# 2gunsu/monocon-pytorch

Hardware: AMD Instinct MI355X
Metric: images/sec (384x1280) fwd+bwd (higher is better)
Workload: dtype f32 (f16x2); 1 GPU; train step B=32/GPU 3x384x1280 (configs[2] shape, fp32 values, mode f16x2); global_batch=32, parallelism=dp1, precision_mode=f16x2

## Files before the change

### monocon-pytorch_amd/csrc/conv_mfma.h

```cpp
#pragma once
#include <hip/hip_runtime.h>
#include <stdint.h>
#include <atomic>
#include <type_traits>
#include <utility>

namespace mc {

typedef float f32x16 __attribute__((ext_vector_type(16)));
typedef float f32x4 __attribute__((ext_vector_type(4)));

struct DynLdsOnce {
    std::atomic<unsigned long long> done{0};
    hipError_t ensure(const void *fn, int bytes) {
        int dev = 0;
        if (hipGetDevice(&dev) != hipSuccess || dev < 0 || dev >= 64) return hipFuncSetAttribute(fn, hipFuncAttributeMaxDynamicSharedMemorySize, bytes);
        if ((done.load(std::memory_order_acquire) >> dev) & 1ull) return hipSuccess;
        const hipError_t e = hipFuncSetAttribute(fn, hipFuncAttributeMaxDynamicSharedMemorySize, bytes);
        if (e == hipSuccess) done.fetch_or(1ull << dev, std::memory_order_release);
        return e;
    }
};

struct ConvSrc {
// ... 324 lines not shown
        if (s.id == (cfg & CFG_SHAPE_BITS)) return s;
    return {0, 0, 0, 0, 0};
}
template <int I>
struct ConvShapeC {
    static constexpr int WM = CONV_SHAPES[I].WM, WN = CONV_SHAPES[I].WN, WTM = CONV_SHAPES[I].WTM, WTN = CONV_SHAPES[I].WTN;
    static constexpr int PB = CONV_SHAPES[I].PB(), BNT = CONV_SHAPES[I].BNT();
};
template <typename F, int... I>
inline hipError_t with_conv_shape_seq(int id, F &f, std::integer_sequence<int, I...>) {
    hipError_t e = hipErrorInvalidValue;
    (void)((CONV_SHAPES[I].id == id && ((e = f(ConvShapeC<I>{})), true)) || ...);
    return e;
}
template <typename F>
inline hipError_t with_conv_shape(int cfg, F &&f) {
    return with_conv_shape_seq(cfg & CFG_SHAPE_BITS, f, std::make_integer_sequence<int, CONV_NSHAPES>{});
}
template <int KS_, int S_>
struct ConvWin { static constexpr int KS = KS_, S = S_; };
template <typename F>
inline hipError_t with_conv_window(int ks, int stride, F &&f) {
    if (ks == 3 && stride == 1) return f(ConvWin<3, 1>{});
    if (ks == 3 && stride == 2) return f(ConvWin<3, 2>{});
    if (stride != 1) return hipErrorInvalidValue;
    if (ks == 1) return f(ConvWin<1, 1>{});
    if (ks == 12) return f(ConvWin<12, 1>{});
    if (ks == 21) return f(ConvWin<21, 1>{});
    if (ks == 22) return f(ConvWin<22, 1>{});
    return hipErrorInvalidValue;
}

template <auto Kern, typename... Args>
inline hipError_t launch_dyn_lds(size_t lds_bytes, dim3 grid, dim3 block, hipStream_t st, const Args &...args) {
    if (lds_bytes > 160 * 1024) return hipErrorInvalidValue;
    static DynLdsOnce attr_set;
    const hipError_t e = attr_set.ensure(reinterpret_cast<const void *>(Kern), (int)lds_bytes);
    if (e != hipSuccess) return e;
    hipLaunchKernelGGL(Kern, grid, block, lds_bytes, st, args...);
    return hipGetLastError();
}

inline int conv_ntile(int Cout) { return Cout >= 128 ? 128 : (Cout > 32 ? 64 : 32); }
inline int conv_coutp(int Cout) {
    const int t = conv_ntile(Cout);
    return (Cout + t - 1) / t * t;
}
inline int conv_out_dim(int in, int ks, int stride) { return (in + 2 * (ks / 2) - ks) / stride + 1; }
inline int split_pieces(int prec) { return prec == 2 ? 3 : (prec == 3 ? 2 : 1); }
inline int conv_ck(int ks, int stride, const int *src_c, int nsrc) {
    bool all32 = true;
    for (int i = 0; i < nsrc; ++i) all32 = all32 && (src_c[i] % 32 == 0);
    if (ks == 3 && stride == 2) return 16;
    return all32 ? 32 : 16;
}
int conv_pick_cfg(int Cout, int CoutP, int ks, int stride, int B, int Hout, int Wout);
inline int conv_chunks_per_image(int cfg, int Hout, int Wout) {
    if (cfg == CFG_SMALL) return Hout;
    return ((Wout + 7) / 8) * ((Hout + 3) / 4);
}
inline void conv_set_patches(ConvArgs &a, int PB) {
    a.ppr = (a.Wout + 7) / 8;
    a.ppi = a.ppr * ((a.Hout + 3) / 4);
    a.chunks = (a.ppi + PB - 1) / PB;
}
inline bool any_lazy_src(const ConvSrc *src, int nsrc) {
    for (int i = 0; i < nsrc; ++i)
        if (src[i].la) return true;
    return false;
}
inline bool conv_any_lazy(const ConvArgs &a) { return any_lazy_src(a.src, a.nsrc); }
bool conv_small_ok(const ConvArgs &a, int ks, int stride);
bool conv_small_lazy_ok(const ConvArgs &a, int ks, int stride);
bool conv_bf16_ok(const ConvArgs &a, int ks, int stride);
hipError_t launch_conv_bf16(const ConvArgs &a, int ks, int stride, hipStream_t st, ConvArgs *resolved);
hipError_t launch_absmax(const float *x, size_t n, unsigned *slot, hipStream_t st, bool single_word = false);
bool conv_wres_ok(const ConvArgs &a, int ks, int stride);
hipError_t launch_conv_wres(const ConvArgs &a, int ks, int stride, hipStream_t st, ConvArgs *resolved);
hipError_t launch_conv_small(const ConvArgs &a, int stride, hipStream_t st);
bool conv_thin_ok(const ConvArgs &a, int ks, int stride);
hipError_t launch_conv_thin(const ConvArgs &a, hipStream_t st);
bool dgrad_s2_thin_ok(int prec, int ks, int stride, int dyC, int srcC, int CinTotal, int c_off, const unsigned *amax_dy,
                      const unsigned *amax_w, int H, int W);
hipError_t launch_dgrad_s2_thin(const float *dy, int B, int H, int W, int dyC, const float *w_master, int CinTotal, int c_off, float *out,
                                int accumulate, const unsigned *amax_dy, const unsigned *amax_w, hipStream_t st);

hipError_t launch_conv(const ConvArgs &a, int ks, int stride, hipStream_t st, ConvArgs *resolved = nullptr);
bool conv_lazy_capable(const ConvArgs &a, int ks, int stride);

struct ProfLast { int kind; double flops, bytes; };
extern thread_local ProfLast prof_last;

}
```

### monocon-pytorch_amd/csrc/conv_thin.hip

```cpp
#include "conv_mfma.h"
#include "train.h"

#ifndef THIN_OCC
#define THIN_OCC 2
#endif
#ifndef THIN_MT_UNROLL
#define THIN_MT_UNROLL 1
#endif
namespace mc {

typedef _Float16 f16x8 __attribute__((ext_vector_type(8)));
typedef _Float16 f16x4 __attribute__((ext_vector_type(4)));
typedef float f32x4v __attribute__((ext_vector_type(4)));

namespace {
constexpr int TR = 8, TW = 64;
constexpr int IR = TR + 2, IP = TW + 2;
constexpr int PLANE = IR * IP * 16;
constexpr int ITEMS = IR * IP * 4;
constexpr int NI = (ITEMS + 255) / 256;
}

template <int NTN>
__global__ __launch_bounds__(256, THIN_OCC) void conv_thin16_kernel(const ConvArgs a) {
// ... 175 lines not shown
                            const unsigned char *p = lds + half * PLANE + ((trow + r) * IP + mt * 16 + li + c) * 16;
                            ah = *reinterpret_cast<const f16x8 *>(p);
                            al = *reinterpret_cast<const f16x8 *>(p + 2 * PLANE);
                        }
#pragma unroll
                        for (int nt = 0; nt < NTN; ++nt) {
                            accm[nt] = __builtin_amdgcn_mfma_f32_16x16x32_f16(al, bw[s][0][nt], accm[nt], 0, 0, 0);
                            accm[nt] = __builtin_amdgcn_mfma_f32_16x16x32_f16(ah, bw[s][1][nt], accm[nt], 0, 0, 0);
                            acc[nt] = __builtin_amdgcn_mfma_f32_16x16x32_f16(ah, bw[s][0][nt], acc[nt], 0, 0, 0);
                        }
                    }
#pragma unroll
                    for (int nt = 0; nt < NTN; ++nt) {
                        const int n = nt * 16 + li;
                        const int v_out = nok[nt] ? ((4 * kq) * a.out_ld + a.out_coff + n) * 4 : BUF_OOB;
                        const int v_res = nok[nt] ? ((4 * kq) * a.res_ld + n) * 4 : BUF_OOB;
                        float rv[4];
                        if (has_res) {
#pragma unroll
                            for (int e = 0; e < 4; ++e) rv[e] = buf_load1(r_res[q], v_res, (x0 + e) * a.res_ld * 4);
                        }
#pragma unroll
                        for (int e = 0; e < 4; ++e) {
                            float v = ((accm[nt][e] + acc[nt][e]) * omul) * sc[nt] + bi[nt];
                            if (has_res) v += rv[e];
                            if (bm) {
                                if (rok && nok[nt]) {
                                    const float yv = ybm[nt][e];
                                    const bool on = bm_relu == 0 || (bm_relu == 1 ? zbm[nt][e] > 0.f : fmaf(yv, ma[nt], mb[nt]) > 0.f);
                                    v = on ? v : 0.f;
                                    ssum[q][nt] += v;
                                    ssq[q][nt] = fmaf(v, yv, ssq[q][nt]);
                                }
                            } else if (do_stats) {
                                const float d = v - sh[nt];
                                ssum[q][nt] += d;
                                ssq[q][nt] += d * d;
                            }
                            v = fmaxf(v, floor_v);
                            vmax = fmaxf(vmax, (nok[nt] && oy0 + trow < a.Hout) ? fabsf(v) : 0.f);
                            buf_store1(v, r_out[q], v_out, (x0 + e) * a.out_ld * 4);
                        }
                    }
                }
            }
        }
        if (do_stats) {
#pragma unroll
            for (int q = 0; q < 2; ++q) {
                const int oy = oy0 + 2 * wave + q;
                if (oy >= a.Hout) continue;
#pragma unroll
                for (int nt = 0; nt < NTN; ++nt) {
                    float s1 = ssum[q][nt], s2 = ssq[q][nt];
                    s1 += __shfl_xor(s1, 16); s2 += __shfl_xor(s2, 16);
                    s1 += __shfl_xor(s1, 32); s2 += __shfl_xor(s2, 32);
                    if (kq == 0 && nok[nt]) {
                        float *dst = a.stats + (((size_t)img * a.Hout + oy) * a.CoutP + nt * 16 + li) * 2;
                        dst[0] = s1;
                        dst[1] = s2;
                    }
                }
            }
        }
    }
    if (a.amax_out) amax_update_wave(a.amax_out, vmax);
}

bool conv_thin_ok(const ConvArgs &a, int ks, int stride) {
#ifdef MC_NO_CONV_THIN
    return false;
#endif
    return a.prec == 3 && ks == 3 && stride == 1 && a.nsrc == 1 && a.Cin == 16 && a.Cout == 16 && a.amax_in[0] && a.amax_w &&
           a.Wout % 16 == 0 && a.Hout == a.Hin && a.Wout == a.Win && a.CoutP >= 16;
}

hipError_t launch_conv_thin(const ConvArgs &a, hipStream_t st) {
    const int tiles = a.B * ((a.Hout + TR - 1) / TR);
    hipLaunchKernelGGL((conv_thin16_kernel<1>), dim3(tiles < 4096 ? tiles : 4096), dim3(256), 0, st, a);
    return hipGetLastError();
}


struct DgradS2Args {
    const float *dy;
    const float *w;
    float *out;
    int B, H, W, CinTotal, c_off, accumulate;
    const unsigned *amax_dy, *amax_w;
};
namespace {
constexpr int DR = 4, DW = 32;
constexpr int DIR_ = DR + 1, DIP = DW + 1;
constexpr int DPLANE = DIR_ * DIP * 16;
}
template <int KS, int NT>
__global__ __launch_bounds__(256, KS == 1 ? 2 : 1) void dgrad_s2_thin_kernel(const DgradS2Args a) {
    constexpr int CY = 32 * KS, CX = 16 * NT, NOCT = 4 * KS;
    constexpr int DITEMS = DIR_ * DIP * (CY / 4), DNI = (DITEMS + 255) / 256;
    __shared__ __attribute__((aligned(16))) unsigned char lds[2 * NOCT * DPLANE];
    const int tid = threadIdx.x, lane = tid & 63;
    const int wave = __builtin_amdgcn_readfirstlane(tid >> 6);
    const int li = lane & 15, kq = lane >> 4;
    const int nt = wave % NT, row0 = (wave / NT) * NT;
    const int ex = f16_scale_exp(amax_read(a.amax_dy)), ew = f16_scale_exp(*a.amax_w);
    const float x_scale = exp2i(ex), w_scale = exp2i(ew), omul = exp2i(-ex) * exp2i(-ew);
    f16x8 bw[9][KS][2];
#pragma unroll
    for (int tap = 0; tap < 9; ++tap)
#pragma unroll
        for (int ks = 0; ks < KS; ++ks) {
            f16x8 h8, l8;
#pragma unroll
            for (int q = 0; q < 8; ++q) {
                const float ws = a.w[((size_t)(32 * ks + 8 * kq + q) * a.CinTotal + a.c_off + 16 * nt + li) * 9 + tap] * w_scale;
                const _Float16 hh = (_Float16)ws;
                h8[q] = hh;
                l8[q] = (_Float16)(ws - (float)hh);
            }
            bw[tap][ks][0] = h8; bw[tap][ks][1] = l8;
        }
    int s_off[DNI], s_dst[DNI];
#pragma unroll
    for (int i = 0; i < DNI; ++i) {
        const int e = tid + 256 * i;
        const int c4 = e % (CY / 4), px = (e / (CY / 4)) % DIP, row = (e / (CY / 4)) / DIP;
        s_off[i] = ((row * a.W + px) * CY + c4 * 4) * 4;
        s_dst[i] = e < DITEMS ? (c4 >> 1) * DPLANE + (row * DIP + px) * 16 + (c4 & 1) * 8 : -1;
    }
    const int tiles_per_img = (a.H + DR - 1) / DR, nstrips = (a.W + DW - 1) / DW;
    const int Ho = 2 * a.H, Wo = 2 * a.W;
    for (int tile = xcd_order(blockIdx.x, gridDim.x); tile < a.B * tiles_per_img; tile += gridDim.x) {
        const int img = tile / tiles_per_img, i0 = (tile - img * tiles_per_img) * DR;
        const __amdgpu_buffer_rsrc_t r_x = make_rsrc(a.dy + (size_t)img * a.H * a.W * CY, (unsigned)(a.H * a.W * CY) * 4u);
        __amdgpu_buffer_rsrc_t r_out[NT][2];
#pragma unroll
        for (int rr = 0; rr < NT; ++rr)
#pragma unroll
            for (int py = 0; py < 2; ++py) {
                const int i = i0 + row0 + rr;
                const bool ok = i < a.H;
                r_out[rr][py] = make_rsrc(a.out + ((size_t)img * Ho + (ok ? 2 * i + py : 0)) * Wo * CX, ok ? (unsigned)(Wo * CX) * 4u : 0u);
            }
        f32x4 pre[DNI];
        auto fetch = [&](int strip) {
            const int j0 = strip * DW, so = (i0 * a.W + j0) * CY * 4;
#pragma unroll
            for (int k = 0; k < DNI; ++k) {
                const int px = ((s_dst[k] % DPLANE) >> 4) % DIP;
                const bool ok = s_dst[k] >= 0 && j0 + px < a.W;
                pre[k] = buf_load4(r_x, ok ? s_off[k] + so : BUF_OOB, 0);
            }
        };
        fetch(0);
        for (int strip = 0; strip < nstrips; ++strip) {
            __syncthreads();
#pragma unroll
            for (int k = 0; k < DNI; ++k) {
                if (256 * (k + 1) > DITEMS && s_dst[k] < 0) continue;
                f16x4 h4, l4;
#pragma unroll
                for (int q = 0; q < 4; ++q) {
                    const float xs = pre[k][q] * x_scale;
                    const _Float16 hh = (_Float16)xs;
                    h4[q] = hh;
                    l4[q] = (_Float16)(xs - (float)hh);
                }
                *reinterpret_cast<f16x4 *>(lds + s_dst[k]) = h4;
                *reinterpret_cast<f16x4 *>(lds + NOCT * DPLANE + s_dst[k]) = l4;
            }
            __syncthreads();
            if (strip + 1 < nstrips) fetch(strip + 1);
            const int j0 = strip * DW;
#pragma unroll
            for (int rr = 0; rr < NT; ++rr) {
#pragma unroll
                for (int mt = 0; mt < DW / 16; ++mt) {
                    if (j0 + mt * 16 >= a.W) break;
#pragma unroll
                    for (int py = 0; py < 2; ++py) {
#pragma unroll
                        for (int px = 0; px < 2; ++px) {
                            f32x4v acc = {0.f, 0.f, 0.f, 0.f}, accm = {0.f, 0.f, 0.f, 0.f};
#pragma unroll
                            for (int dr = 0; dr <= py; ++dr) {
#pragma unroll
                                for (int ds = 0; ds <= px; ++ds) {
                                    const int r = py ? 2 - 2 * dr : 1, sx = px ? 2 - 2 * ds : 1, tap = r * 3 + sx;
#pragma unroll
                                    for (int ks = 0; ks < KS; ++ks) {
                                        const unsigned char *p = lds + (ks * 4 + kq) * DPLANE + ((row0 + rr + dr) * DIP + mt * 16 + li + ds) * 16;
                                        const f16x8 ah = *reinterpret_cast<const f16x8 *>(p), al = *reinterpret_cast<const f16x8 *>(p + NOCT * DPLANE);
                                        accm = __builtin_amdgcn_mfma_f32_16x16x32_f16(al, bw[tap][ks][0], accm, 0, 0, 0);
                                        accm = __builtin_amdgcn_mfma_f32_16x16x32_f16(ah, bw[tap][ks][1], accm, 0, 0, 0);
                                        acc = __builtin_amdgcn_mfma_f32_16x16x32_f16(ah, bw[tap][ks][0], acc, 0, 0, 0);
                                    }
                                }
                            }
#pragma unroll
                            for (int e = 0; e < 4; ++e) {
                                const int j = j0 + mt * 16 + 4 * kq + e;
                                const int voff = j < a.W ? ((2 * j + px) * CX + 16 * nt + li) * 4 : BUF_OOB;
                                float v = (accm[e] + acc[e]) * omul;
                                if (a.accumulate) v += buf_load1(r_out[rr][py], voff, 0);
                                buf_store1(v, r_out[rr][py], voff, 0);
                            }
                        }
                    }
                }
            }
        }
    }
}
bool dgrad_s2_thin_ok(int prec, int ks, int stride, int dyC, int srcC, int CinTotal, int c_off, const unsigned *amax_dy,
                      const unsigned *amax_w, int H, int W) {
    const bool shape = dyC == 32 && srcC == 16;
    return prec == 3 && ks == 3 && stride == 2 && shape && c_off >= 0 && c_off + srcC <= CinTotal && amax_dy && amax_w &&
           (size_t)H * W * dyC * 4 < (1ull << 31) && (size_t)4 * W * srcC * 4 < (1ull << 31);
}
hipError_t launch_dgrad_s2_thin(const float *dy, int B, int H, int W, int dyC, const float *w_master, int CinTotal, int c_off, float *out,
                                int accumulate, const unsigned *amax_dy, const unsigned *amax_w, hipStream_t st) {
    DgradS2Args a;
    a.dy = dy; a.w = w_master; a.out = out; a.B = B; a.H = H; a.W = W; a.CinTotal = CinTotal; a.c_off = c_off;
    a.accumulate = accumulate; a.amax_dy = amax_dy; a.amax_w = amax_w;
    const int tiles = B * ((H + DR - 1) / DR);
    const int srcC = dyC / 2;
    prof_last = {1, 2.0 * B * H * W * (double)dyC * srcC * 9.0, 4.0 * ((double)B * H * W * dyC + (double)B * 4 * H * W * srcC * (accumulate ? 2 : 1))};
    if (dyC != 32) return hipErrorInvalidValue;
    hipLaunchKernelGGL((dgrad_s2_thin_kernel<1, 1>), dim3(tiles < 4096 ? tiles : 4096), dim3(256), 0, st, a);
    return hipGetLastError();
}

namespace {
constexpr int WT_XT = 128, WT_P = 152, WT_ROWS = 6;
constexpr int WT_PLANE = 16 * WT_ROWS * WT_P * 2;
typedef unsigned u32x4 __attribute__((ext_vector_type(4)));
typedef _Float16 f16x2 __attribute__((ext_vector_type(2)));
}

__global__ __launch_bounds__(256) void wgrad_thin16_kernel(const WgradArgs a) {
    extern __shared__ __attribute__((aligned(16))) unsigned char wsm[];
    unsigned char *win = wsm;
    float (*red)[64] = reinterpret_cast<float (*)[64]>(wsm + 2 * WT_PLANE);
    const int tid = threadIdx.x, lane = tid & 63;
    const int wave = __builtin_amdgcn_readfirstlane(tid >> 6);
    const int g = lane >> 4, j = lane & 15;
    const int ex = f16_scale_exp(amax_read(a.amax_x[0])), ed = f16_scale_exp(amax_read(a.amax_dy));
    const float x_scale = exp2i(ex), d_scale = exp2i(ed), omul = exp2i(-ex) * exp2i(-ed);
    const int H = a.Hout, W = a.Wout;
    const bool lazy = a.src[0].la != nullptr;
    f32x4 lzA = {0.f, 0.f, 0.f, 0.f}, lzB = lzA;
    if (lazy) {
        lzA = reinterpret_cast<const f32x4 *>(a.src[0].la)[tid & 3];
        lzB = reinterpret_cast<const f32x4 *>(a.src[0].lb)[tid & 3];
#pragma unroll
        for (int q = 0; q < 4; ++q) { lzA[q] *= x_scale; lzB[q] *= x_scale; }
    }
    const unsigned x_bytes = (unsigned)(a.Hin * a.Win * 16) * 4u;
    unsigned okm = 0u;

    f32x4v acc[9], accm[9];
#pragma unroll
    for (int t = 0; t < 9; ++t) { acc[t] = f32x4v{0.f, 0.f, 0.f, 0.f}; accm[t] = f32x4v{0.f, 0.f, 0.f, 0.f}; }
    const int va = (8 * g * 16 + j) * 4;
    const int boff = ((j * WT_ROWS + wave) * WT_P + 8 * g) * 2;

    constexpr int NITEM = WT_ROWS * (WT_P / 2) * 4, NIW = (NITEM + 255) / 256;
    int w_off[NIW], w_dst[NIW];
#pragma unroll
    for (int i = 0; i < NIW; ++i) {
        const int e = tid + 256 * i, c4 = e & 3, pr = (e >> 2) % (WT_P / 2), row = (e >> 2) / (WT_P / 2);
        w_off[i] = ((row * a.Win + 2 * pr) * 16 + c4 * 4) * 4;
        w_dst[i] = e < NITEM ? ((c4 * 4 * WT_ROWS + row) * WT_P + 2 * pr) * 2 : -1;
    }
    const int tiles_x = (W + WT_XT - 1) / WT_XT, tiles_y = (H + 3) / 4;
    const int ntiles = a.B * tiles_y * tiles_x;
    f32x4 pv[NIW][2];
    auto fetch = [&](int tl) {
        const int b = tl / (tiles_y * tiles_x), rem = tl - b * tiles_y * tiles_x;
        const int y0 = (rem / tiles_x) * 4, x0 = (rem % tiles_x) * WT_XT;
        const __amdgpu_buffer_rsrc_t r_x = make_rsrc(a.src[0].p + (size_t)b * a.Hin * a.Win * 16, (unsigned)(a.Hin * a.Win * 16) * 4u);
        const int so = ((y0 - 1) * a.Win + x0 - 1) * 64;
        okm = 0u;
#pragma unroll
        for (int i = 0; i < NIW; ++i) {
            const int col = x0 - 1 + ((w_dst[i] >> 1) % WT_P);
            const bool live = w_dst[i] >= 0;
            const int vo0 = (live && col >= 0 && col < a.Win) ? w_off[i] + so : BUF_OOB;
            const int vo1 = (live && col + 1 >= 0 && col + 1 < a.Win) ? w_off[i] + so + 64 : BUF_OOB;
            pv[i][0] = buf_load4(r_x, vo0, 0);
            pv[i][1] = buf_load4(r_x, vo1, 0);
            if (lazy) okm |= (((unsigned)vo0 < x_bytes ? 1u : 0u) | ((unsigned)vo1 < x_bytes ? 2u : 0u)) << (2 * i);
        }
    };
    float araw[WT_XT / 32][8];
    auto fetch_dy = [&](int tl, float (&dst)[WT_XT / 32][8]) {
        const int b = tl / (tiles_y * tiles_x), rem = tl - b * tiles_y * tiles_x;
        const int y = (rem / tiles_x) * 4 + wave, x0 = (rem % tiles_x) * WT_XT;
        const __amdgpu_buffer_rsrc_t r_dy =
            make_rsrc(a.dy + ((size_t)b * H + (y < H ? y : 0)) * W * a.dy_ld, y < H ? (unsigned)(W * a.dy_ld) * 4u : 0u);
#pragma unroll
        for (int G = 0; G < WT_XT / 32; ++G)
#pragma unroll
            for (int t = 0; t < 8; ++t) dst[G][t] = buf_load1(r_dy, va + t * 64, (x0 + G * 32) * 64);
    };
    if ((int)blockIdx.x < ntiles) { fetch(blockIdx.x); fetch_dy(blockIdx.x, araw); }
    for (int tl = blockIdx.x; tl < ntiles; tl += gridDim.x) {
        __syncthreads();
#pragma unroll
        for (int i = 0; i < NIW; ++i) {
            if (w_dst[i] < 0) continue;
            const float cap0 = ((okm >> (2 * i)) & 1u) ? __builtin_inff() : 0.f, cap1 = ((okm >> (2 * i + 1)) & 1u) ? __builtin_inff() : 0.f;
// ... 94 lines not shown
```

### monocon-pytorch_amd/csrc/mc_train_plan.hip

```cpp
#include <atomic>
#include <deque>
#include <functional>

#include "mc_internal.h"

using namespace mc;

namespace {

using Fn = std::function<int(mc_handle *, hipStream_t)>;

struct PlanSwitches {
    long long lazy_z;
    long long lazy_min;
    long long lazy_feat;
    long long zbits;
    long long grad_pool;
    long long grad_pool_cool;
    long long head_dx_fuse;
    long long head_zskip;
    long long dgrad_s2_thin;
    long long stem_fuse;
    long long bm_epilogue;
    long long wres_bwd;
    long long dual_stream;
    int side_sync_lo = 0, side_sync_hi = 0;
    bool plan_debug = false;
};
const struct { const char *name; long long PlanSwitches::*field; long long def; } SWITCH_TABLE[] = {
    {"MONOCON_HIP_LAZY_Z", &PlanSwitches::lazy_z, 3},
    {"MONOCON_HIP_LAZY_MIN", &PlanSwitches::lazy_min, 900000},
    {"MONOCON_HIP_LAZY_FEAT", &PlanSwitches::lazy_feat, 0},
    {"MONOCON_HIP_ZBITS", &PlanSwitches::zbits, 1},
    {"MONOCON_HIP_GRAD_POOL", &PlanSwitches::grad_pool, 1},
    {"MONOCON_HIP_GRAD_POOL_COOL", &PlanSwitches::grad_pool_cool, 2},
    {"MONOCON_HIP_HEAD_DX_FUSE", &PlanSwitches::head_dx_fuse, 1},
    {"MONOCON_HIP_HEAD_ZSKIP", &PlanSwitches::head_zskip, 1},
    {"MONOCON_HIP_DGRAD_S2_THIN", &PlanSwitches::dgrad_s2_thin, 1},
    {"MONOCON_HIP_STEM_FUSE", &PlanSwitches::stem_fuse, 1},
    {"MONOCON_HIP_BM_EPILOGUE", &PlanSwitches::bm_epilogue, 1},
    {"MONOCON_HIP_WRES_BWD", &PlanSwitches::wres_bwd, 0},
    {"MONOCON_HIP_DUAL_STREAM", &PlanSwitches::dual_stream, 1},
};
PlanSwitches read_switches() {
    PlanSwitches sw{};
    std::string changed;
    for (const auto &d : SWITCH_TABLE) {
        const char *e = std::getenv(d.name);
        sw.*d.field = e ? std::atoll(e) : d.def;
        if (sw.*d.field != d.def) changed += std::string(" ") + d.name + "=" + std::to_string(sw.*d.field);
    }
    if (const char *e = std::getenv("MONOCON_HIP_SIDE_SYNC")) {
        if (std::sscanf(e, "%d:%d", &sw.side_sync_lo, &sw.side_sync_hi) != 2) sw.side_sync_lo = sw.side_sync_hi = 0;
        if (sw.side_sync_lo < sw.side_sync_hi) changed += std::string(" MONOCON_HIP_SIDE_SYNC=") + e;
    }
    sw.plan_debug = std::getenv("MONOCON_HIP_PLAN_DEBUG") != nullptr;
    if (sw.plan_debug && !changed.empty()) fprintf(stderr, "[plan] switches off their defaults:%s\n", changed.c_str());
    return sw;
}

struct PoolBwdArgs {
    const float *x, *dout, *la, *lb;
    float *dx, *stats;
    int B, H, W, C, acc;
};

struct LastWriter {
    enum Kind { NONE, DGRAD_CONV, POOL_BWD, DECONV_BWD } kind = NONE;
    union {
        ConvArgs *conv;
        PoolBwdArgs *pool;
        float **deconv_stats;
    };
    LastWriter() : conv(nullptr) {}
    LastWriter(ConvArgs *c) : kind(c ? DGRAD_CONV : NONE), conv(c) {}
    LastWriter(PoolBwdArgs *p) : kind(p ? POOL_BWD : NONE), pool(p) {}
    LastWriter(float **s) : kind(s ? DECONV_BWD : NONE), deconv_stats(s) {}
};

struct TNode {
    Tensor t;
    float *g = nullptr;
    bool ginit = false, needs_grad = true;
    LastWriter last;
};

enum RecKind { REC_STEM, REC_CONV, REC_POOL, REC_DECONV, REC_HEAD };
struct Rec {
    RecKind kind;
    ConvLayer *L = nullptr;
    DeconvLayer *D = nullptr;
    std::vector<int> srcs;
    int res = -1, z = -1, in = -1;
    bool relu = true, dead = false;
    Tensor y;
    float *mean = nullptr, *rstd = nullptr;
    float *ca = nullptr, *cb = nullptr;
    unsigned *zbits = nullptr;
    std::string bn;
};

enum BwdStream { ON_MAIN, ON_SIDE };
struct BwdStep {
    Fn fn;
    BwdStream stream = ON_MAIN;
    int wait = -1;
    int bucket = -1;
    bool feat_dgrad = false;
    bool img_dgrad = false;
    hipEvent_t ready = nullptr;
    hipEvent_t fin = nullptr;
};

}

struct TrainState {
    int B = 0, H = 0, W = 0;
    unsigned long long bind_gen = 0;
    PlanSwitches sw{};
    PlanMem mem;
    std::vector<TNode> nodes;
    std::vector<Rec> recs;
    std::vector<Fn> fwd;
    std::vector<BwdStep> bwd;
    std::deque<ConvArgs> dgrads;
    std::deque<PoolBwdArgs> pool_bwds;
    std::deque<float *> deconv_stats;
    hipStream_t side = nullptr;
    hipEvent_t side_done = nullptr;
    bool dual = true;
    unsigned *img_amax = nullptr;
    mc::PackBatch pack_batch;
    std::vector<Fn> pack_fns;
    const float *img = nullptr;
    mc_labels labels{};
    float *preds[10] = {nullptr};
    float *losses = nullptr;
    const float *grad_losses = nullptr;
    const float *grad_preds[10] = {nullptr};
    int pad_h = 0, pad_w = 0, max_objs = 30;
    bool head_only = false;
    const float *feat_ext = nullptr;
    float *gfeat_ext = nullptr;
    bool skip_feat_dgrad = false;
    float *gimg_ext = nullptr;
    mc_targets targets{};
    float *dpred[10] = {nullptr};
    bool ok = true;
};

static std::atomic<unsigned long long> g_train_generation{0};

static void train_free(TrainState *t) {
    if (!t) return;
    for (const BwdStep &s : t->bwd) {
        if (s.ready) (void)hipEventDestroy(s.ready);
        if (s.fin) (void)hipEventDestroy(s.fin);
    }
    if (t->side_done) (void)hipEventDestroy(t->side_done);
    if (t->side) (void)hipStreamDestroy(t->side);
    t->mem.release();
    delete t;
}

namespace {

struct TB {
    mc_handle *h;
    TrainState *ts;
    PlanAlloc mem{h, ts->mem, ts->ok, 1, 1024};
    const PlanSwitches &sw = ts->sw;
    const int B = ts->B, H = ts->H, W = ts->W, fh = H / 4, fw = W / 4, HW = fh * fw;

    float *alloc(size_t n) { return mem.alloc(n); }
    unsigned *slot() { return mem.slot(); }
    unsigned *w_slot(const float *w_master) {
        if (h->prec != 3) return nullptr;
        auto it = h->w_amax_of.find(w_master);
        if (it == h->w_amax_of.end()) { ts->ok = false; h->err = "train plan: no max-|w| slot for a master weight"; return nullptr; }
        return it->second;
    }

    int cur_bucket = 0;
    int pending_wait = -1;
    int push_bwd(Fn fn, BwdStream stream = ON_MAIN) {
        BwdStep s;
        s.fn = std::move(fn); s.stream = stream; s.bucket = cur_bucket; s.wait = pending_wait;
        pending_wait = -1;
        ts->bwd.push_back(std::move(s));
        return (int)ts->bwd.size() - 1;
    }

    struct PoolBuf { float *p; int side_step; };
    std::map<size_t, std::deque<PoolBuf>> gpool;
    float *g_acquire(int node) {
        TNode &n = ts->nodes[node];
        if (n.g) return n.g;
        const size_t ne = n.t.numel();
        auto &q = gpool[ne];
        if (sw.grad_pool && (long long)q.size() > sw.grad_pool_cool) {
            const PoolBuf b = q.front();
            q.pop_front();
            pending_wait = std::max(pending_wait, b.side_step);
            n.g = b.p;
        } else {
            n.g = alloc(ne);
        }
        return n.g;
// ... 167 lines not shown
        r.y.p = alloc(r.y.numel());
        const bool lazy = !dead && !never_lazy && res < 0 && h->prec == 3 && (sw.lazy_z & (relu ? 1 : 2)) != 0 &&
                          (!relu || s.elementwise_consumers || (long long)Ho * Wo * Lr.cout >= sw.lazy_min);
        r.z = dead ? -1 : node(B, Ho, Wo, Lr.cout, true, !lazy);
        ConvArgs a{};
        const std::vector<const Tensor *> xs = conv_sources(srcs);
        if (!conv_fwd_args(a, Lr, xs, h->prec)) { ts->ok = false; h->err = "train plan: channel mismatch at " + Lr.conv; }
        if (conv_any_lazy(a) && !conv_lazy_capable(a, Lr.ks, Lr.stride)) {
            for (int s_ : srcs) materialise(s_);
            conv_fwd_args(a, Lr, xs, h->prec);
        }
        a.out = r.y.p; a.out_ld = Lr.cout;
        unsigned *yslot = lazy ? slot() : nullptr;
        a.amax_out = yslot;
        a.cfg = ts->ok ? mc_choose_conv_cfg(h, a, Lr.ks, Lr.stride) : CFG_128x32;
        const int chunks = conv_chunks_per_image(a.cfg, Ho, Wo);
        float *stats = alloc((size_t)B * chunks * Lr.coutp * 2);
        a.stats = stats;
        a.stat_shift = P(Lr.bn + ".running_mean", Lr.cout);
        const int ks = Lr.ks, stride = Lr.stride;
        ts->fwd.push_back([=](mc_handle *hh, hipStream_t st) { HIPCHK(hh, launch_conv(a, ks, stride, st)); return 0; });
        bn_act(r, stats, B * chunks, Lr.coutp, lazy, yslot);
        ts->recs.push_back(r);
        return r.z;
    }

    int pool(int x) {
        const Tensor t = ts->nodes[x].t;
        if (ts->nodes[x].t.la && !ts->nodes[x].t.lrelu) materialise(x);
        const Tensor tx = ts->nodes[x].t;
        const int o = node(t.B, t.H / 2, t.W / 2, t.C, true);
        ts->nodes[o].t.amax = t.amax;
        const float *ip = tx.p, *la = tx.la, *lb = tx.lb;
        float *op = ts->nodes[o].t.p;
        const int B = t.B, H = t.H, W = t.W, C = t.C;
        ts->fwd.push_back([=](mc_handle *hh, hipStream_t st) {
            HIPCHK(hh, launch_maxpool2(ip, B, H, W, C, op, st, la, lb));
            return 0;
        });
        Rec r;
        r.kind = REC_POOL; r.in = x; r.z = o;
        ts->recs.push_back(r);
        return o;
    }

    int deconv(DeconvLayer &D, int x) {
        if (ts->nodes[x].t.la && !ts->nodes[x].t.lrelu) materialise(x);
        const Tensor t = ts->nodes[x].t;
        const int o = node(t.B, t.H * 2, t.W * 2, t.C, true);
        const float *ip = t.p, *w = D.wpk, *la = t.la, *lb = t.lb;
        float *op = ts->nodes[o].t.p;
        unsigned *omax = ts->nodes[o].t.amax;
        const int B = t.B, H = t.H, W = t.W, C = t.C;
        ts->fwd.push_back([=](mc_handle *hh, hipStream_t st) {
            HIPCHK(hh, launch_deconv4(ip, B, H, W, C, w, op, st, omax, la, lb));
            return 0;
        });
        Rec r;
        r.kind = REC_DECONV; r.in = x; r.z = o; r.D = &D;
        ts->recs.push_back(r);
        return o;
    }

    const PackJobDesc &pack_job(const float *w, int Cout, int CinTotal, int k, int c_off, int Cs, int CoutPad, int cls) {
        const size_t pn = dgrad_panel_elems(k, cls, CoutPad, Cs);
        float *dst = alloc(pn);
        void *dst16 = panel_has_pieces(h->prec, CoutPad) ? alloc((3 * pn + 1) / 2) : nullptr;
        ts->pack_batch.add(pack_job_dgrad(w, Cout, CinTotal, k, c_off, Cs, CoutPad, cls, dst, dst16, h->prec, w_slot(w)));
        return ts->pack_batch.jobs.back();
    }

    void emit_dgrad(const float *w_master, const Tensor &dy, int Cout_fwd, int CinTotal, int ks, int stride, int c_off, int srcnode,
                    int CoutPad) {
        TNode &sn = ts->nodes[srcnode];
        if (!sn.needs_grad) return;
        g_acquire(srcnode);
        auto dgrad_conv = [&](int cls, ConvArgs &d) {
            const PackJobDesc &p = pack_job(w_master, Cout_fwd, CinTotal, ks, c_off, sn.t.C, CoutPad, cls);
            return dgrad_conv_args(d, p, h->prec, dy.p, dy.amax, dy.B, dy.H, dy.W, dy.C, sn.g, sn.t.H, sn.t.W, sn.ginit);
        };
        if (stride == 2 && ks == 3) {
            if (2 * dy.H != sn.t.H || 2 * dy.W != sn.t.W) { ts->ok = false; h->err = "train plan: stride-2 dgrad shape mismatch"; }
            if (sw.dgrad_s2_thin && ts->ok && dgrad_s2_thin_ok(h->prec, ks, stride, dy.C, sn.t.C, CinTotal, c_off, dy.amax, w_slot(w_master), dy.H, dy.W)) {
                const float *dyp = dy.p;
                float *gp = sn.g;
                const int B = dy.B, Hd = dy.H, Wd = dy.W, Cd = dy.C, acc = sn.ginit ? 1 : 0;
                const unsigned *dmax = dy.amax, *wmax = w_slot(w_master);
                push_bwd([=](mc_handle *hh, hipStream_t st) {
                    HIPCHK(hh, launch_dgrad_s2_thin(dyp, B, Hd, Wd, Cd, w_master, CinTotal, c_off, gp, acc, dmax, wmax, st));
                    return 0;
                });
                wrote(srcnode);
                return;
            }
            for (int cls = 0; cls < 4; ++cls) {
                ConvArgs d;
                const int kk = dgrad_conv(cls, d);
                d.cfg = ts->ok ? mc_choose_conv_cfg(h, d, kk, 1) : CFG_128x32;
                push_bwd([=](mc_handle *hh, hipStream_t st) { HIPCHK(hh, launch_conv(d, kk, 1, st)); return 0; });
            }
            wrote(srcnode);
            return;
        }
        ConvArgs d;
        dgrad_conv(-1, d);
        if (dy.H != sn.t.H || dy.W != sn.t.W) { ts->ok = false; h->err = "train plan: dgrad shape mismatch"; }
        d.cfg = ts->ok ? mc_choose_conv_cfg(h, d, ks, 1) : CFG_128x32;
        if (sw.wres_bwd < 2) d.cfg &= ~CFG_WRES;
        ts->dgrads.push_back(d);
        ConvArgs *dp = &ts->dgrads.back();
        push_bwd([=](mc_handle *hh, hipStream_t st) { HIPCHK(hh, launch_conv(*dp, ks, 1, st)); return 0; });
        wrote(srcnode, (d.cfg == CFG_SMALL && !conv_thin_ok(d, ks, 1)) ? nullptr : dp);
    }

    int emit_wgrad(const std::vector<int> &srcs, const Tensor &dy, int dy_ld, int Cout, int ks, int stride, float *dw) {
        WgradArgs a{};
        const std::vector<const Tensor *> xs = conv_sources(srcs);
        wgrad_args(a, xs, dy, dy_ld, Cout, ks, stride, h->prec);
        if (wgrad_any_lazy(a) && !wgrad_lazy_capable(a, ks, stride)) {
            for (int s_ : srcs) materialise(s_);
            wgrad_args(a, xs, dy, dy_ld, Cout, ks, stride, h->prec);
        }
        a.partial = alloc(wgrad_partial_floats(a, ks));
        return push_bwd([=](mc_handle *hh, hipStream_t st) { HIPCHK(hh, launch_wgrad(a, ks, stride, dw, st)); return 0; }, ON_SIDE);
    }

    struct BnBwd { Tensor dy; float *coef; bool affine_skipped; };
    BnBwd bn_backward(const Rec &r, const std::string &bn, bool caller_forms_dy = false) {
        TNode &zn = ts->nodes[r.z];
        Tensor dy = r.y;
        dy.p = zn.g;
        dy.amax = slot();
        unsigned *dymax = dy.amax;
        const int B = r.y.B, C = r.y.C, rows = r.y.H * r.y.W;
        const float *yp = r.y.p, *gz = zn.g, *zp = zn.t.p, *gamma = P(bn + ".weight", C), *mean = r.mean, *rstd = r.rstd;
        float *dg = G(bn + ".weight", C), *db = G(bn + ".bias", C), *dyp = dy.p;
        float *coef = alloc((size_t)C * 4);
        const int relu = r.relu ? ((r.res < 0 && r.ca && r.cb) ? 2 : 1) : 0;
        const float *fa = r.ca, *fb = r.cb;
        float *gres = nullptr;
        int gmode = 0;
        if (r.res >= 0 && ts->nodes[r.res].needs_grad) {
            gres = g_acquire(r.res);
            gmode = ts->nodes[r.res].ginit ? 2 : 1;
            wrote(r.res);
        }
        const double n = (double)B * rows;
        auto step = [&](float *partial, int nbp, int cstride, bool reduce, bool affine) {
            double *fold = fold_scratch(nbp, C);
            const int arelu = reduce ? relu : 0;
            const float *aa = reduce ? fa : nullptr, *ab = reduce ? fb : nullptr;
            push_bwd([=](mc_handle *hh, hipStream_t st) {
                if (reduce) HIPCHK(hh, launch_chan_reduce(yp, gz, zp, nullptr, B, rows, C, 1, relu, partial, C, st, fa, fb));
                HIPCHK(hh, launch_bn_bwd_finalize(partial, nbp, cstride, n, C, gamma, mean, rstd, dg, db, coef, st, fold));
                if (affine)
                    HIPCHK(hh, launch_affine_bwd(gz, zp, yp, coef, B, (size_t)rows, C, 0, arelu, dyp, gres, gmode, st, aa, ab, nullptr,
                                                 nullptr, dymax));
                return 0;
            });
            return BnBwd{dy, coef, !affine};
        };
        const LastWriter last = zn.last;
        ConvArgs *lc = last.kind == LastWriter::DGRAD_CONV ? last.conv : nullptr;
        if (sw.bm_epilogue == 0 || (sw.bm_epilogue > 1 && r.y.H * r.y.W > sw.bm_epilogue)) lc = nullptr;
        if (sw.plan_debug)
            fprintf(stderr, "[plan] bn_backward %-40s %4d ch %4dx%-4d relu %d res %d last-writer-conv %d\n", bn.c_str(), C, r.y.H,
                    r.y.W, relu, r.res >= 0, lc != nullptr);
        if (lc && lc->out == zn.g && lc->Cout == C && lc->out_ld == C && lc->Hout == r.y.H && lc->Wout == r.y.W && !lc->stats) {
            const int ppi = conv_chunks_per_image(lc->cfg, r.y.H, r.y.W), nbp = B * ppi, cstride = lc->CoutP;
            float *partial = alloc((size_t)nbp * cstride * 2);
            lc->stats = partial;
            lc->bm_y = yp; lc->bm_z = zp; lc->bm_a = fa; lc->bm_b = fb; lc->bm_relu = relu;
            lc->bm_zbits = relu == 1 ? r.zbits : nullptr;
            if (sw.wres_bwd >= 1 && !(lc->cfg & (CFG_SMALL | CFG_WS)) && conv_wres_ok(*lc, 3, 1)) lc->cfg |= CFG_WRES;
            if (sw.plan_debug)
                fprintf(stderr, "[plan]   twin of %-36s cfg %3d  K %4d  Cout %3d  %dx%d  res %d  nsrc %d srcC %d wres %d\n", bn.c_str(), lc->cfg,
                        lc->Cin, lc->Cout, lc->Hout, lc->Wout, lc->res != nullptr, lc->nsrc, lc->src[0].C, (lc->cfg & CFG_WRES) != 0);
            const bool skip_affine = caller_forms_dy && !gres;
            if (skip_affine) lc->amax_out = dymax;
            return step(partial, nbp, cstride, false, !skip_affine);
        }
        PoolBwdArgs *pl = last.kind == LastWriter::POOL_BWD ? last.pool : nullptr;
        if (pl && relu == 2 && pl->la == fa && pl->lb == fb && pl->x == yp && pl->acc && pl->dx == zn.g && pl->C == C &&
            pl->H * pl->W == rows && !pl->stats && !caller_forms_dy && C % 4 == 0 && 256 % (C / 4) == 0) {
            const int nbp = maxpool2_bwd_blocks(B, pl->H, pl->W, C);
            float *partial = alloc((size_t)nbp * C * 2);
            pl->stats = partial;
            if (sw.plan_debug)
                fprintf(stderr, "[plan]   statistics of %-36s left by the max-pool backward (%d partial rows)\n", bn.c_str(), nbp);
            return step(partial, nbp, C, false, true);
        }
        float **ds = last.kind == LastWriter::DECONV_BWD ? last.deconv_stats : nullptr;
        if (ds && relu == 2 && zn.t.la == fa && zn.t.lb == fb && !*ds && !caller_forms_dy && !gres) {
            const int nbp = B * r.y.H;
            float *partial = alloc((size_t)nbp * C * 2);
            *ds = partial;
            if (sw.plan_debug)
                fprintf(stderr, "[plan]   statistics of %-36s left by the deconv backward (%d partial rows)\n", bn.c_str(), nbp);
            return step(partial, nbp, C, false, true);
        }
        const int nb = chan_reduce_blocks(B, rows);
        return step(alloc((size_t)nb * C * 2), nb, C, true, true);
    }

    static constexpr int CP = NUM_HEADS * HEAD_CH, LD = 80;
    Tensor xh;
    AttnTrainArgs at{};
    AttnGradPtrs gp{};
    float *w3dense = nullptr;
    size_t raw_numel = 0;

    void heads_forward(int feat) {
        xh.B = B; xh.H = fh; xh.W = fw; xh.C = CP; xh.p = alloc(xh.numel());
        Tensor raw; raw.B = B; raw.H = fh; raw.W = fw; raw.C = LD; raw.p = alloc(raw.numel());
        raw_numel = raw.numel();
        for (int hd = 0; hd < NUM_HEADS; ++hd) {
            const std::string an = mc_head_keys(hd).attn;
            const int A = NUM_AFFINE, AC = NUM_AFFINE * HEAD_CH;
            at.rm[hd] = P(an + ".running_mean", HEAD_CH); at.rv[hd] = P(an + ".running_var", HEAD_CH);
            at.nbt[hd] = NBT(an + ".num_batches_tracked");
            at.att_w[hd] = P(an + ".attn_weights.attention.0.weight", AC);
            at.att_g[hd] = P(an + ".attn_weights.attention.1.weight", A);
            at.att_b[hd] = P(an + ".attn_weights.attention.1.bias", A);
            at.att_rm[hd] = P(an + ".attn_weights.attention.1.running_mean", A);
            at.att_rv[hd] = P(an + ".attn_weights.attention.1.running_var", A);
            at.att_nbt[hd] = NBT(an + ".attn_weights.attention.1.num_batches_tracked");
            at.weight_[hd] = P(an + ".weight_", AC); at.bias_[hd] = P(an + ".bias_", AC);
            gp.d_weight_[hd] = G(an + ".weight_", AC); gp.d_bias_[hd] = G(an + ".bias_", AC);
            gp.d_att_w[hd] = G(an + ".attn_weights.attention.0.weight", AC);
            gp.d_att_g[hd] = G(an + ".attn_weights.attention.1.weight", A);
            gp.d_att_b[hd] = G(an + ".attn_weights.attention.1.bias", A);
        }
        ConvArgs c3{};
        at.chunks = mc_head_conv_args(h, mem, ts->nodes[feat].t, xh.p, c3);
        if (conv_any_lazy(c3) && (!ts->nodes[feat].t.lrelu || !conv_lazy_capable(c3, 3, 1))) {
            materialise(feat);
            conv_fwd_args(c3, h->head3, {&ts->nodes[feat].t}, h->prec);
        }
        at.stat_ld = h->head3.coutp;
        at.stats = c3.stats; at.B = B; at.HW = HW;
        at.stats64 = reinterpret_cast<double *>(alloc((size_t)B * at.stat_ld * 4));
        at.sv_inst = alloc((size_t)B * CP * 3); at.mu_r = alloc((size_t)CP * 2); at.bn10 = alloc(NUM_HEADS * NUM_AFFINE * 2);
        at.that = alloc((size_t)B * NUM_HEADS * NUM_AFFINE); at.yatt = alloc((size_t)B * NUM_HEADS * NUM_AFFINE);
        at.gamma_p = alloc((size_t)B * CP); at.scale = alloc((size_t)B * CP); at.shift = alloc((size_t)B * CP);
        w3dense = alloc((size_t)CP * 64 * 9);
        HeadApplyArgs ha{};
        ha.hidden = xh.p; ha.scale = at.scale; ha.shift = at.shift; ha.w = h->head_w1t; ha.b = h->head_b1;
        ha.B = B; ha.HW = HW; ha.z_out = nullptr;
        for (int i = 0; i < 10; ++i) ha.pred_c[i] = PRED_CH[i];
        ts->fwd.push_back([=](mc_handle *hh, hipStream_t st) { HIPCHK(hh, launch_conv(c3, 3, 1, st)); return 0; });
        ts->fwd.push_back([=, ts = ts, at = at](mc_handle *hh, hipStream_t st) {
            HIPCHK(hh, launch_attn_train_fwd(at, st));
            HeadApplyArgs a2 = ha;
            for (int i = 0; i < 10; ++i) a2.pred[i] = ts->preds[i];
            HIPCHK(hh, launch_head_apply(a2, st));
            return 0;
        });
    }

    void targets_and_losses() {
        mc_targets &T = ts->targets;
        const size_t R = (size_t)B * ts->max_objs;
        auto up = [](size_t n) { return (n + 63) / 64 * 64; };
        const size_t tn[15] = {(size_t)B * 3 * HW, (size_t)B * 9 * HW, R * 2, R * 2, R * 3, R, R, R, R * 18, R * 18,
// ... 522 lines not shown
```

### scratch/plan_fingerprint.py

```python
import hashlib, json, os, sys
import numpy as np
import torch
REPO = os.path.dirname(os.path.dirname(os.path.abspath(__file__)))
for p in (os.path.join(REPO, "monocon-pytorch_amd"), REPO):
    sys.path.insert(0, p)
from hipmonocon import synth
from model import MonoConDetector
from solver import AdamW

mode = sys.argv[1] if len(sys.argv) > 1 else "f16x2"
stats = np.load(os.path.join(REPO, "tests", "golden", "bn_calib_seed7.npz"))


def digest(named):
    h = hashlib.sha256()
    for name, t in named:
        h.update(name.encode())
        h.update(t.detach().cpu().contiguous().numpy().tobytes())
    return h.hexdigest()


def run(B, H, W):
    sd = synth.make_state_dict(7, bn_stats={k: stats[k] for k in stats.files})
    m = MonoConDetector(34, pretrained_backbone=False)
    m.load_state_dict(sd, strict=True)
    m = m.cuda().train().set_precision(mode)
    opt = AdamW(m.parameters(), lr=2.25e-4, weight_decay=1e-5, betas=(0.95, 0.99), max_grad_norm=35.0)
    b = synth.make_batch(500, B, H, W)
    bt = {"img": b["img"].cuda().contiguous(), "label": {k: v.cuda().contiguous() for k, v in b["label"].items()},
          "img_metas": {"pad_shape": [(H, W)] * B}}
    losses, grads = [], None
    for step in range(2):
        opt.zero_grad()
        _, loss = m(bt)
        sum(loss.values()).backward()
        torch.cuda.synchronize()
        losses += [("%d.%s" % (step, k), v) for k, v in sorted(loss.items())]
        if step == 0:
            grads = digest((n, p.grad) for n, p in m.named_parameters() if p.grad is not None)
        opt.step()
    torch.cuda.synchronize()
    return {"shape": [B, H, W], "workspace_bytes": m._rt.engine.workspace_bytes(), "losses": digest(losses), "grads_step1": grads,
            "state_step2": digest(sorted(m.state_dict().items()))}


switches = {k: v for k, v in sorted(os.environ.items()) if k.startswith("MONOCON_HIP_") and k != "MONOCON_HIP_TUNE_CACHE"}
print(json.dumps({"mode": mode, "switches": switches, "runs": [run(4, 128, 224), run(2, 384, 1280)]}, sort_keys=True))
```

Measured before the change: 675.6 images/sec.

## Fuse BN-backward statistics and ReLU mask into stride-2 thin dgrad epilogue

Extends the stride-2 thin data-gradient kernel with an optional epilogue that applies the following batch-norm/ReLU mask and accumulates per-row partial sums for the BN backward statistics. The train planner records the stride-2 dgrad as a last writer so the BN backward can reuse its partial stats instead of launching a separate reduction pass over the gradient. This removes one full read of a large high-resolution gradient tensor. In exchange the kernel now reads the forward activation and keeps extra registers, which may lower occupancy.

```diff
diff --git a/monocon-pytorch_amd/csrc/conv_mfma.h b/monocon-pytorch_amd/csrc/conv_mfma.h
--- a/monocon-pytorch_amd/csrc/conv_mfma.h
+++ b/monocon-pytorch_amd/csrc/conv_mfma.h
@@ -430,8 +430,16 @@
 hipError_t launch_conv_thin(const ConvArgs &a, hipStream_t st);
 bool dgrad_s2_thin_ok(int prec, int ks, int stride, int dyC, int srcC, int CinTotal, int c_off, const unsigned *amax_dy,
                       const unsigned *amax_w, int H, int W);
-hipError_t launch_dgrad_s2_thin(const float *dy, int B, int H, int W, int dyC, const float *w_master, int CinTotal, int c_off, float *out,
-                                int accumulate, const unsigned *amax_dy, const unsigned *amax_w, hipStream_t st);
+struct DgradS2Args {
+    const float *dy;
+    const float *w;
+    float *out;
+    int B, H, W, dyC, CinTotal, c_off, accumulate;
+    const unsigned *amax_dy, *amax_w;
+    const float *bm_y = nullptr, *bm_a = nullptr, *bm_b = nullptr;
+    float *stats = nullptr;
+};
+hipError_t launch_dgrad_s2_thin(const DgradS2Args &a, hipStream_t st);
 
 hipError_t launch_conv(const ConvArgs &a, int ks, int stride, hipStream_t st, ConvArgs *resolved = nullptr);
 bool conv_lazy_capable(const ConvArgs &a, int ks, int stride);
diff --git a/monocon-pytorch_amd/csrc/conv_thin.hip b/monocon-pytorch_amd/csrc/conv_thin.hip
--- a/monocon-pytorch_amd/csrc/conv_thin.hip
+++ b/monocon-pytorch_amd/csrc/conv_thin.hip
@@ -281,19 +281,12 @@
 }
 
 
-struct DgradS2Args {
-    const float *dy;
-    const float *w;
-    float *out;
-    int B, H, W, CinTotal, c_off, accumulate;
-    const unsigned *amax_dy, *amax_w;
-};
 namespace {
 constexpr int DR = 4, DW = 32;
 constexpr int DIR_ = DR + 1, DIP = DW + 1;
 constexpr int DPLANE = DIR_ * DIP * 16;
 }
-template <int KS, int NT>
+template <int KS, int NT, bool BM>
 __global__ __launch_bounds__(256, KS == 1 ? 2 : 1) void dgrad_s2_thin_kernel(const DgradS2Args a) {
     constexpr int CY = 32 * KS, CX = 16 * NT, NOCT = 4 * KS;
     constexpr int DITEMS = DIR_ * DIP * (CY / 4), DNI = (DITEMS + 255) / 256;
@@ -329,10 +322,12 @@
     }
     const int tiles_per_img = (a.H + DR - 1) / DR, nstrips = (a.W + DW - 1) / DW;
     const int Ho = 2 * a.H, Wo = 2 * a.W;
+    const float ma = BM ? a.bm_a[16 * nt + li] : 0.f, mb = BM ? a.bm_b[16 * nt + li] : 0.f;
     for (int tile = xcd_order(blockIdx.x, gridDim.x); tile < a.B * tiles_per_img; tile += gridDim.x) {
         const int img = tile / tiles_per_img, i0 = (tile - img * tiles_per_img) * DR;
         const __amdgpu_buffer_rsrc_t r_x = make_rsrc(a.dy + (size_t)img * a.H * a.W * CY, (unsigned)(a.H * a.W * CY) * 4u);
-        __amdgpu_buffer_rsrc_t r_out[NT][2];
+        __amdgpu_buffer_rsrc_t r_out[NT][2], r_y[NT][2];
+        float ssum[NT][2], ssq[NT][2];
 #pragma unroll
         for (int rr = 0; rr < NT; ++rr)
 #pragma unroll
@@ -340,6 +335,8 @@
                 const int i = i0 + row0 + rr;
                 const bool ok = i < a.H;
                 r_out[rr][py] = make_rsrc(a.out + ((size_t)img * Ho + (ok ? 2 * i + py : 0)) * Wo * CX, ok ? (unsigned)(Wo * CX) * 4u : 0u);
+                if (BM) r_y[rr][py] = make_rsrc(a.bm_y + ((size_t)img * Ho + (ok ? 2 * i + py : 0)) * Wo * CX, ok ? (unsigned)(Wo * CX) * 4u : 0u);
+                ssum[rr][py] = ssq[rr][py] = 0.f;
             }
         f32x4 pre[DNI];
         auto fetch = [&](int strip) {
@@ -376,8 +373,21 @@
 #pragma unroll
                 for (int mt = 0; mt < DW / 16; ++mt) {
                     if (j0 + mt * 16 >= a.W) break;
+                    float ybm[2][2][4];
+                    if (BM) {
+#pragma unroll
+                        for (int py = 0; py < 2; ++py)
+#pragma unroll
+                            for (int px = 0; px < 2; ++px)
+#pragma unroll
+                                for (int e = 0; e < 4; ++e) {
+                                    const int j = j0 + mt * 16 + 4 * kq + e;
+                                    ybm[py][px][e] = buf_load1(r_y[rr][py], j < a.W ? ((2 * j + px) * CX + 16 * nt + li) * 4 : BUF_OOB, 0);
+                                }
+                    }
 #pragma unroll
                     for (int py = 0; py < 2; ++py) {
+                        float m1[2] = {0.f, 0.f}, m2[2] = {0.f, 0.f};
 #pragma unroll
                         for (int px = 0; px < 2; ++px) {
                             f32x4v acc = {0.f, 0.f, 0.f, 0.f}, accm = {0.f, 0.f, 0.f, 0.f};
@@ -396,18 +406,46 @@
                                     }
                                 }
                             }
+                            float vd[4];
 #pragma unroll
                             for (int e = 0; e < 4; ++e) {
                                 const int j = j0 + mt * 16 + 4 * kq + e;
                                 const int voff = j < a.W ? ((2 * j + px) * CX + 16 * nt + li) * 4 : BUF_OOB;
                                 float v = (accm[e] + acc[e]) * omul;
                                 if (a.accumulate) v += buf_load1(r_out[rr][py], voff, 0);
+                                if (BM) v = (j < a.W && i0 + row0 + rr < a.H && fmaf(ybm[py][px][e], ma, mb) > 0.f) ? v : 0.f;
+                                vd[e] = v;
                                 buf_store1(v, r_out[rr][py], voff, 0);
                             }
+                            if (BM) {
+                                const float *yv = ybm[py][px];
+                                m1[px] = (vd[0] + vd[1]) + (vd[2] + vd[3]);
+                                m2[px] = fmaf(vd[1], yv[1], vd[0] * yv[0]) + fmaf(vd[3], yv[3], vd[2] * yv[2]);
+                            }
+                        }
+                        if (BM) {
+                            ssum[rr][py] += m1[0] + m1[1];
+                            ssq[rr][py] += m2[0] + m2[1];
                         }
                     }
                 }
             }
+        }
+        if (BM) {
+#pragma unroll
+            for (int rr = 0; rr < NT; ++rr)
+#pragma unroll
+                for (int py = 0; py < 2; ++py) {
+                    float s1 = ssum[rr][py], s2 = ssq[rr][py];
+                    s1 += __shfl_xor(s1, 16); s2 += __shfl_xor(s2, 16);
+                    s1 += __shfl_xor(s1, 32); s2 += __shfl_xor(s2, 32);
+                    const int i = i0 + row0 + rr;
+                    if (kq == 0 && i < a.H) {
+                        float *dst = a.stats + (((size_t)img * Ho + 2 * i + py) * CX + 16 * nt + li) * 2;
+                        dst[0] = s1;
+                        dst[1] = s2;
+                    }
+                }
         }
     }
 }
@@ -417,16 +455,18 @@
     return prec == 3 && ks == 3 && stride == 2 && shape && c_off >= 0 && c_off + srcC <= CinTotal && amax_dy && amax_w &&
            (size_t)H * W * dyC * 4 < (1ull << 31) && (size_t)4 * W * srcC * 4 < (1ull << 31);
 }
-hipError_t launch_dgrad_s2_thin(const float *dy, int B, int H, int W, int dyC, const float *w_master, int CinTotal, int c_off, float *out,
-                                int accumulate, const unsigned *amax_dy, const unsigned *amax_w, hipStream_t st) {
-    DgradS2Args a;
-    a.dy = dy; a.w = w_master; a.out = out; a.B = B; a.H = H; a.W = W; a.CinTotal = CinTotal; a.c_off = c_off;
-    a.accumulate = accumulate; a.amax_dy = amax_dy; a.amax_w = amax_w;
+hipError_t launch_dgrad_s2_thin(const DgradS2Args &a, hipStream_t st) {
+    const int B = a.B, H = a.H, W = a.W, dyC = a.dyC;
     const int tiles = B * ((H + DR - 1) / DR);
     const int srcC = dyC / 2;
-    prof_last = {1, 2.0 * B * H * W * (double)dyC * srcC * 9.0, 4.0 * ((double)B * H * W * dyC + (double)B * 4 * H * W * srcC * (accumulate ? 2 : 1))};
-    if (dyC != 32) return hipErrorInvalidValue;
-    hipLaunchKernelGGL((dgrad_s2_thin_kernel<1, 1>), dim3(tiles < 4096 ? tiles : 4096), dim3(256), 0, st, a);
+    const bool bm = a.bm_y != nullptr;
+    prof_last = {1, 2.0 * B * H * W * (double)dyC * srcC * 9.0,
+                 4.0 * ((double)B * H * W * dyC + (double)B * 4 * H * W * srcC * ((a.accumulate ? 2 : 1) + (bm ? 1 : 0)))};
+    if (dyC != 32 || (bm && !(a.bm_a && a.bm_b && a.stats))) return hipErrorInvalidValue;
+    if (bm)
+        hipLaunchKernelGGL((dgrad_s2_thin_kernel<1, 1, true>), dim3(tiles < 4096 ? tiles : 4096), dim3(256), 0, st, a);
+    else
+        hipLaunchKernelGGL((dgrad_s2_thin_kernel<1, 1, false>), dim3(tiles < 4096 ? tiles : 4096), dim3(256), 0, st, a);
     return hipGetLastError();
 }
 
diff --git a/monocon-pytorch_amd/csrc/mc_train_plan.hip b/monocon-pytorch_amd/csrc/mc_train_plan.hip
--- a/monocon-pytorch_amd/csrc/mc_train_plan.hip
+++ b/monocon-pytorch_amd/csrc/mc_train_plan.hip
@@ -21,6 +21,7 @@
     long long head_zskip;
     long long dgrad_s2_thin;
     long long stem_fuse;
+    long long front_bwd;
     long long bm_epilogue;
     long long wres_bwd;
     long long dual_stream;
@@ -38,6 +39,7 @@
     {"MONOCON_HIP_HEAD_ZSKIP", &PlanSwitches::head_zskip, 1},
     {"MONOCON_HIP_DGRAD_S2_THIN", &PlanSwitches::dgrad_s2_thin, 1},
     {"MONOCON_HIP_STEM_FUSE", &PlanSwitches::stem_fuse, 1},
+    {"MONOCON_HIP_FRONT_BWD", &PlanSwitches::front_bwd, 1},
     {"MONOCON_HIP_BM_EPILOGUE", &PlanSwitches::bm_epilogue, 1},
     {"MONOCON_HIP_WRES_BWD", &PlanSwitches::wres_bwd, 0},
     {"MONOCON_HIP_DUAL_STREAM", &PlanSwitches::dual_stream, 1},
@@ -66,14 +68,16 @@
 };
 
 struct LastWriter {
-    enum Kind { NONE, DGRAD_CONV, POOL_BWD, DECONV_BWD } kind = NONE;
+    enum Kind { NONE, DGRAD_CONV, DGRAD_S2, POOL_BWD, DECONV_BWD } kind = NONE;
     union {
         ConvArgs *conv;
+        DgradS2Args *s2;
         PoolBwdArgs *pool;
         float **deconv_stats;
     };
     LastWriter() : conv(nullptr) {}
     LastWriter(ConvArgs *c) : kind(c ? DGRAD_CONV : NONE), conv(c) {}
+    LastWriter(DgradS2Args *d) : kind(d ? DGRAD_S2 : NONE), s2(d) {}
     LastWriter(PoolBwdArgs *p) : kind(p ? POOL_BWD : NONE), pool(p) {}
     LastWriter(float **s) : kind(s ? DECONV_BWD : NONE), deconv_stats(s) {}
 };
@@ -124,6 +128,7 @@
     std::vector<Fn> fwd;
     std::vector<BwdStep> bwd;
     std::deque<ConvArgs> dgrads;
+    std::deque<DgradS2Args> dgrad_s2s;
     std::deque<PoolBwdArgs> pool_bwds;
     std::deque<float *> deconv_stats;
     hipStream_t side = nullptr;
@@ -457,15 +462,14 @@
         if (stride == 2 && ks == 3) {
             if (2 * dy.H != sn.t.H || 2 * dy.W != sn.t.W) { ts->ok = false; h->err = "train plan: stride-2 dgrad shape mismatch"; }
             if (sw.dgrad_s2_thin && ts->ok && dgrad_s2_thin_ok(h->prec, ks, stride, dy.C, sn.t.C, CinTotal, c_off, dy.amax, w_slot(w_master), dy.H, dy.W)) {
-                const float *dyp = dy.p;
-                float *gp = sn.g;
-                const int B = dy.B, Hd = dy.H, Wd = dy.W, Cd = dy.C, acc = sn.ginit ? 1 : 0;
-                const unsigned *dmax = dy.amax, *wmax = w_slot(w_master);
-                push_bwd([=](mc_handle *hh, hipStream_t st) {
-                    HIPCHK(hh, launch_dgrad_s2_thin(dyp, B, Hd, Wd, Cd, w_master, CinTotal, c_off, gp, acc, dmax, wmax, st));
-                    return 0;
-                });
-                wrote(srcnode);
+                DgradS2Args d{};
+                d.dy = dy.p; d.w = w_master; d.out = sn.g;
+                d.B = dy.B; d.H = dy.H; d.W = dy.W; d.dyC = dy.C; d.CinTotal = CinTotal; d.c_off = c_off; d.accumulate = sn.ginit ? 1 : 0;
+                d.amax_dy = dy.amax; d.amax_w = w_slot(w_master);
+                ts->dgrad_s2s.push_back(d);
+                DgradS2Args *dp = &ts->dgrad_s2s.back();
+                push_bwd([=](mc_handle *hh, hipStream_t st) { HIPCHK(hh, launch_dgrad_s2_thin(*dp, st)); return 0; });
+                wrote(srcnode, (sw.front_bwd & 1) ? dp : nullptr);
                 return;
             }
             for (int cls = 0; cls < 4; ++cls) {
@@ -555,6 +559,17 @@
             if (skip_affine) lc->amax_out = dymax;
             return step(partial, nbp, cstride, false, !skip_affine);
         }
+        DgradS2Args *s2 = last.kind == LastWriter::DGRAD_S2 ? last.s2 : nullptr;
+        if (sw.bm_epilogue == 0 || (sw.bm_epilogue > 1 && r.y.H * r.y.W > sw.bm_epilogue)) s2 = nullptr;
+        if (s2 && relu == 2 && s2->out == zn.g && s2->dyC == 2 * C && 2 * s2->H == r.y.H && 2 * s2->W == r.y.W && s2->B == B && !s2->stats) {
+            const int nbp = B * r.y.H;
+            float *partial = alloc((size_t)nbp * C * 2);
+            s2->stats = partial;
+            s2->bm_y = yp; s2->bm_a = fa; s2->bm_b = fb;
+            if (sw.plan_debug)
+                fprintf(stderr, "[plan]   statistics of %-36s left by the stride-2 data gradient (%d partial rows)\n", bn.c_str(), nbp);
+            return step(partial, nbp, C, false, true);
+        }
         PoolBwdArgs *pl = last.kind == LastWriter::POOL_BWD ? last.pool : nullptr;
         if (pl && relu == 2 && pl->la == fa && pl->lb == fb && pl->x == yp && pl->acc && pl->dx == zn.g && pl->C == C &&
             pl->H * pl->W == rows && !pl->stats && !caller_forms_dy && C % 4 == 0 && 256 % (C / 4) == 0) {
diff --git a/scratch/plan_fingerprint.py b/scratch/plan_fingerprint.py
--- a/scratch/plan_fingerprint.py
+++ b/scratch/plan_fingerprint.py
@@ -8,6 +8,14 @@
 from model import MonoConDetector
 from solver import AdamW
 
+SETTINGS = (("fp32", {}), ("bf16x3", {}), ("f16x2", {})) + tuple(("f16x2", {"MONOCON_HIP_" + k: v}) for k, v in (
+    ("BM_EPILOGUE", "0"), ("DGRAD_S2_THIN", "0"), ("DUAL_STREAM", "0"), ("FRONT_BWD", "0"), ("GRAD_POOL", "0"), ("GRAD_POOL_COOL", "0"),
+    ("HEAD_DX_FUSE", "0"), ("HEAD_ZSKIP", "0"), ("LAZY_FEAT", "1"), ("LAZY_MIN", "0"), ("LAZY_Z", "0"), ("LAZY_Z", "1"), ("STEM_FUSE", "0"),
+    ("WRES_BWD", "1"), ("WRES_BWD", "2"), ("ZBITS", "0")))
+if sys.argv[1:] == ["--settings"]:
+    for md, env in SETTINGS:
+        print(" ".join(["%s=%s" % kv for kv in env.items()] + ["python scratch/plan_fingerprint.py", md]))
+    sys.exit(0)
 mode = sys.argv[1] if len(sys.argv) > 1 else "f16x2"
 stats = np.load(os.path.join(REPO, "tests", "golden", "bn_calib_seed7.npz"))
 
```

Result: no change. 679.2 images/sec (median of 6 runs) (+0.5%).
